# facebookresearch/PoseDiffusion

Measured on NVIDIA H100. Metric: diffusion steps/sec (20-frame seq, GGS on), higher is better.
Workload: dtype f32

## Files before the change

### posediffusion_b200/csrc/api_tc.cu

```cuda
#include <cuda.h>
#include <cudaTypedefs.h>

#include <algorithm>
#include <cstdint>
#include <cstdlib>

#include "context.cuh"
#include "tc_linear.cuh"

using namespace pdb;

namespace {

PFN_cuTensorMapEncodeTiled_v12000 get_encode() {
  static PFN_cuTensorMapEncodeTiled_v12000 fn = nullptr;
  if (!fn) {
    void* p = nullptr;
    cudaDriverEntryPointQueryResult qres;
    if (cudaGetDriverEntryPoint("cuTensorMapEncodeTiled", &p, cudaEnableDefault, &qres) == cudaSuccess &&
        qres == cudaDriverEntryPointSuccess)
      fn = reinterpret_cast<PFN_cuTensorMapEncodeTiled_v12000>(p);
  }
  return fn;
}
// ... 127 lines not shown
  return (long long)(O / 64) * ((S + kTcBM - 1) / kTcBM) <= ctx->sm_count && !getenv("PDB_TC_NO_SMALL");
}

}

extern "C" int pdb_debug_tc_linear(pdb_context* c, const float* x_dev, const float* w_dev, const float* bias_dev,
                                   const float* residual_dev, float* y_dev, int32_t S, int32_t O, int32_t K, int32_t relu,
                                   void* stream) {
  if (!c) return PDB_ERR_INVALID;
  Context* ctx = reinterpret_cast<Context*>(c);
  if (!x_dev || !w_dev || !y_dev) return ctx->fail(PDB_ERR_INVALID, "null argument");
  PDB_CUDA(ctx, cudaSetDevice(ctx->device));
  TcEpilogue E = {};
  E.bias = bias_dev;
  E.residual = residual_dev;
  E.ldr = O;
  E.Y = y_dev;
  E.ldy = O;
  E.S = S;
  E.O = O;
  E.K = K;
  E.relu = relu;
  E.allow_small = 1;
  return enqueue_tc_linear(ctx, x_dev, w_dev, E, static_cast<cudaStream_t>(stream));
}

#include "weights.cuh"

namespace {

__global__ void embed_kernel(const float* __restrict__ x, float* __restrict__ emb, int S) {
  pdl_trigger();
  pdl_wait();
  const int i = blockIdx.x * blockDim.x + threadIdx.x;
  if (i >= S * kPoseEmbPad) return;
  const int s = i / kPoseEmbPad, col = i - s * kPoseEmbPad;
  float v = 0.f;
  if (col < 180) {
    const int j = col < 90 ? col : col - 90;
    const int c = j / 10, k = j - c * 10;
    const float arg = x[s * 9 + c] * (float)(1 << k);
    v = col < 90 ? sinf(arg) : cosf(arg);
  } else if (col < kPoseEmb) {
    v = x[s * 9 + (col - 180)];
  }
  emb[i] = v;
}
__global__ void pivot_add_kernel(float* __restrict__ zproj, const float* __restrict__ w_pivot, int batch, int frames) {
  const int i = blockIdx.x * blockDim.x + threadIdx.x;
  if (i < batch * kDM) zproj[(size_t)(i / kDM) * frames * kDM + (i % kDM)] += w_pivot[i % kDM];
}
__global__ void row_stats_kernel(const float* __restrict__ h, float* __restrict__ mean, float* __restrict__ rstd, int S) {
  pdl_trigger();
  pdl_wait();
  const int row = blockIdx.x * (blockDim.x >> 5) + (threadIdx.x >> 5), lane = threadIdx.x & 31;
  if (row >= S) return;
  const float4* p = reinterpret_cast<const float4*>(h + (size_t)row * kDM);
  float4 v[4];
  float sum = 0.f;
#pragma unroll
  for (int i = 0; i < 4; ++i) {
    v[i] = p[lane + 32 * i];
    sum += v[i].x + v[i].y + v[i].z + v[i].w;
  }
  const float m = warp_sum(sum) * (1.0f / kDM);
  float sq = 0.f;
#pragma unroll
  for (int i = 0; i < 4; ++i) {
    const float a = v[i].x - m, b = v[i].y - m, c = v[i].z - m, d = v[i].w - m;
    sq += a * a + b * b + c * c + d * d;
  }
  const float var = warp_sum(sq) * (1.0f / kDM);
  if (lane == 0) {
    mean[row] = m;
    rstd[row] = 1.0f / sqrtf(var + kLnEps);
  }
}
__global__ void __launch_bounds__(kDenThreads) attention_kernel(const float* __restrict__ qkv, float* __restrict__ att, int frames) {
  extern __shared__ __align__(16) float att_smem[];
  pdl_trigger();
  pdl_wait();
  const int chunks = (frames + kDenWarps - 1) / kDenWarps;
  const int item = blockIdx.x;
  attention_item<false>(att_smem, qkv, att, item / (kHeads * chunks), (item / chunks) % kHeads, item % chunks, frames, 0u, 0u);
}
__global__ void __launch_bounds__(kDenThreads) tail_kernel(const __grid_constant__ DenoiserDev W, const __grid_constant__ DenoiserRun R, const int* __restrict__ tstate) {
  pdl_trigger();
  pdl_wait();
  const int s = blockIdx.x * kDenWarps + (threadIdx.x >> 5);
  const int t = tstate[0];
  if (s < R.tokens) tail_token<false>(W, R, s, t, t == tstate[1], 0u, 0u);
}
__global__ void step_set_kernel(int* tstate, int t, int t_lo) { tstate[0] = t; tstate[1] = t_lo; }
__global__ void step_dec_kernel(int* tstate) {
  pdl_wait();
  tstate[0] -= 1;
}

}

namespace pdb {

int enqueue_denoiser_tc(Context* ctx, DenoiserRun run, cudaStream_t st) {
  const DenoiserWeights* w = ctx->weights;
  const TcWeights& T = w->tc;
  const int S = run.tokens, B = run.batch, N = run.frames;
  const size_t need = sizeof(float) * (denoiser_ws_floats(S) + (size_t)S * (kPoseEmbPad + 2) + 64);
  if (int rc = ensure_buffer(ctx, &ctx->den_ws, &ctx->den_ws_bytes, need)) return rc;
  int* tstate = reinterpret_cast<int*>(ctx->den_ws) + 32;
  float* ws = static_cast<float*>(ctx->den_ws) + 64;
  run.zproj = ws; ws += (size_t)S * kDM;
  run.h = ws;     ws += (size_t)S * kDM;
  run.qkv = ws;   ws += (size_t)S * 3 * kDM;
  run.att = ws;   ws += (size_t)S * kDM;
  run.ff = ws;    ws += (size_t)S * kFF;
  run.u = ws;     ws += (size_t)S * kHid;
  float* emb = ws; ws += (size_t)S * kPoseEmbPad;
  float* mean = ws; ws += S;
  float* rstd = ws;
  bool pdl = false;
  auto lin = [&](const float* X, const float* Wm, int O, int K, const float* bias, const int* t_ptr, const float* residual, int ldr,
                 const float* colsum, float* Y, int relu, cudaStream_t s) {
    TcEpilogue E = {};
    E.bias = bias; E.t_ptr = t_ptr; E.bias_t_stride = kDM; E.residual = residual; E.ldr = ldr;
    E.colsum = colsum; E.row_mean = colsum ? mean : nullptr; E.row_rstd = colsum ? rstd : nullptr;
    E.Y = Y; E.ldy = O; E.S = S; E.O = O; E.K = K; E.relu = relu;
    E.allow_small = 1;
    E.pdl = pdl;
    E.stats = colsum && tc_linear_small(ctx, S, O);
    return enqueue_tc_linear(ctx, X, Wm, E, s);
  };
  const size_t att_smem = sizeof(float) * ((size_t)N * (kHD + 4) + (size_t)N * kHD + 2 * kDenWarps * kHD) + 64;
  size_t& att_attr = ctx->attr_att;
  if (att_smem > att_attr) {
    PDB_CUDA(ctx, cudaFuncSetAttribute(attention_kernel, cudaFuncAttributeMaxDynamicSharedMemorySize, (int)att_smem));
    att_attr = att_smem;
  }
  const int chunks = (N + kDenWarps - 1) / kDenWarps;
  const bool was_profiling = ctx->profiling;
  ScopedTimer total(ctx, st, 1);
  ctx->profiling = false;
  if (run.compute_zproj) {
    if (int rc = lin(run.z, T.wz, kDM, kZ, T.b_first, nullptr, nullptr, 0, nullptr, run.zproj, 0, st)) { ctx->profiling = was_profiling; return rc; }
    pivot_add_kernel<<<(B * kDM + 255) / 256, 256, 0, st>>>(run.zproj, T.w_pivot, B, N);
    ctx->launches += 1;
  }
  const bool stats_qkv = tc_linear_small(ctx, S, 3 * kDM), stats_ff1 = tc_linear_small(ctx, S, kFF);
  auto enqueue_step = [&](cudaStream_t s) -> int {
    pdl = ctx->tc_pdl && S <= 320;
    PDB_CUDA(ctx, launch_chained(embed_kernel, dim3((S * kPoseEmbPad + 255) / 256), dim3(256), 0, s, false, (const float*)run.x, emb, S));
    if (int rc = lin(emb, T.wx, kDM, kPoseEmbPad, T.tproj, tstate, run.zproj, kDM, nullptr, run.h, 0, s)) return rc;
    for (int l = 0; l < kLayers; ++l) {
      const TcLayer& L = T.layer[l];
      if (!stats_qkv) PDB_CUDA(ctx, launch_chained(row_stats_kernel, dim3((S + 7) / 8), dim3(256), 0, s, pdl, (const float*)run.h, mean, rstd, S));
      if (int rc = lin(run.h, L.wqkv, 3 * kDM, kDM, L.bias_qkv, nullptr, nullptr, 0, L.colsum_qkv, run.qkv, 0, s)) return rc;
      PDB_CUDA(ctx, launch_chained(attention_kernel, dim3(B * kHeads * chunks), dim3(kDenThreads), att_smem, s, pdl, (const float*)run.qkv, run.att, N));
      if (int rc = lin(run.att, L.wout, kDM, kDM, L.bout, nullptr, run.h, kDM, nullptr, run.h, 0, s)) return rc;
      if (!stats_ff1) PDB_CUDA(ctx, launch_chained(row_stats_kernel, dim3((S + 7) / 8), dim3(256), 0, s, pdl, (const float*)run.h, mean, rstd, S));
      if (int rc = lin(run.h, L.wff1, kFF, kDM, L.bias_ff1, nullptr, nullptr, 0, L.colsum_ff1, run.ff, 1, s)) return rc;
      if (int rc = lin(run.ff, L.wff2, kDM, kFF, L.bff2, nullptr, run.h, kDM, nullptr, run.h, 0, s)) return rc;
    }
    if (int rc = lin(run.h, T.wlast0, kHid, kDM, T.blast0, nullptr, nullptr, 0, nullptr, run.u, 0, s)) return rc;
    PDB_CUDA(ctx, launch_chained(tail_kernel, dim3((S + kDenWarps - 1) / kDenWarps), dim3(kDenThreads), 0, s, pdl, w->dev, run, (const int*)tstate));
    PDB_CUDA(ctx, launch_chained(step_dec_kernel, dim3(1), dim3(1), 0, s, pdl, tstate));
    pdl = false;
    return PDB_OK;
  };
// ... 63 lines not shown
```

### posediffusion_b200/csrc/common.cuh

```cuda
#pragma once
#include <cuda_runtime.h>
#include <stdint.h>

namespace pdb {

constexpr int kTargetDim = 9;
constexpr int kMaxFrames = 128;

__device__ __forceinline__ float warp_sum(float v) {
#pragma unroll
  for (int o = 16; o > 0; o >>= 1) v += __shfl_xor_sync(0xffffffffu, v, o);
  return v;
}

__device__ __forceinline__ float warp_reduce16(float (&v)[16], int lane) {
  {
    const bool hi = lane & 16;
#pragma unroll
    for (int i = 0; i < 8; ++i) {
      float send = hi ? v[i] : v[i + 8];
      float keep = hi ? v[i + 8] : v[i];
      v[i] = keep + __shfl_xor_sync(0xffffffffu, send, 16);
    }
  }
// ... 11 lines not shown
#pragma unroll
    for (int i = 0; i < 2; ++i) {
      float send = hi ? v[i] : v[i + 2];
      float keep = hi ? v[i + 2] : v[i];
      v[i] = keep + __shfl_xor_sync(0xffffffffu, send, 4);
    }
  }
  {
    const bool hi = lane & 2;
    float send = hi ? v[0] : v[1];
    float keep = hi ? v[1] : v[0];
    v[0] = keep + __shfl_xor_sync(0xffffffffu, send, 2);
  }
  v[0] += __shfl_xor_sync(0xffffffffu, v[0], 1);
  return v[0];
}
__device__ __forceinline__ int warp_reduce16_slot(int lane) {
  return ((lane >> 4) & 1) * 8 + ((lane >> 3) & 1) * 4 + ((lane >> 2) & 1) * 2 + ((lane >> 1) & 1);
}

#if defined(PDB_EMU) && defined(__CUDACC__)
#error "PDB_EMU is the CPU test harness of tests/host/cuda_emu.h; it must never be defined in an nvcc (product) build"
#endif
#ifdef PDB_EMU
inline float4 ld_stream_f4(const float4* p) { return *p; }
inline unsigned ld_acquire_u32(const unsigned* p) {
  sched_yield();
  return __atomic_load_n(p, __ATOMIC_ACQUIRE);
}
inline unsigned ld_relaxed_u32(const unsigned* p) { return __atomic_load_n(p, __ATOMIC_RELAXED); }
inline void red_release_add_u32(unsigned* p, unsigned v) { __atomic_fetch_add(p, v, __ATOMIC_RELEASE); }
inline void st_ll(unsigned long long* p, unsigned bits, unsigned tag) {
  __atomic_store_n(p, ((unsigned long long)tag << 32) | (unsigned long long)bits, __ATOMIC_RELAXED);
}
inline unsigned long long ld_ll(const unsigned long long* p) { return __atomic_load_n(p, __ATOMIC_RELAXED); }
inline void pdl_wait() {}
inline void pdl_trigger() {}
inline void ld_ll2(const unsigned long long* p, unsigned long long& a, unsigned long long& b) {
  a = __atomic_load_n(p, __ATOMIC_RELAXED);
  b = __atomic_load_n(p + 1, __ATOMIC_RELAXED);
}
inline void st_ll2(unsigned long long* p, unsigned bits0, unsigned bits1, unsigned tag) {
  st_ll(p, bits0, tag);
  st_ll(p + 1, bits1, tag);
}
inline void red_pair_add(float* p, float v) {
  unsigned long long* u = reinterpret_cast<unsigned long long*>(p);
  unsigned long long old = __atomic_load_n(u, __ATOMIC_RELAXED);
  for (;;) {
    float f[2];
    memcpy(f, &old, 8);
    f[0] += v;
    f[1] += 1.0f;
    unsigned long long want;
    memcpy(&want, f, 8);
    if (__atomic_compare_exchange_n(u, &old, want, false, __ATOMIC_RELAXED, __ATOMIC_RELAXED)) return;
  }
}
inline float2 ld_pair(const float* p) {
  const unsigned long long w = __atomic_load_n(reinterpret_cast<const unsigned long long*>(p), __ATOMIC_RELAXED);
  float f[2];
  memcpy(f, &w, 8);
  return make_float2(f[0], f[1]);
}
inline void st_pair_zero(float* p) { __atomic_store_n(reinterpret_cast<unsigned long long*>(p), 0ull, __ATOMIC_RELAXED); }
inline void red_add_u64(unsigned long long* p, unsigned long long v) { __atomic_fetch_add(p, v, __ATOMIC_RELAXED); }
inline void fence_gpu() { __atomic_thread_fence(__ATOMIC_SEQ_CST); }
inline void ll_backoff() {
  emu::yield();
  sched_yield();
}
inline uint32_t smem_u32(const void* p) { return emu::shared_addr(p); }
inline void mbar_init(uint32_t bar, uint32_t count) { emu::mbar_init(bar, count); }
inline void mbar_fence_init() {}
inline void mbar_arrive_expect_tx(uint32_t bar, uint32_t bytes) { emu::mbar_arrive_expect_tx(bar, bytes); }
inline bool mbar_try_wait(uint32_t bar, uint32_t parity) { return emu::mbar_try_wait(bar, parity); }
inline void mbar_wait(uint32_t bar, uint32_t parity) {
  while (!mbar_try_wait(bar, parity)) {
  }
}
inline void bulk_copy_g2s(uint32_t dst_smem, const void* src, uint32_t bytes, uint32_t bar) { emu::bulk_copy_g2s(dst_smem, src, bytes, bar); }
inline uint64_t l2_policy_evict_first() { return 0; }
inline void bulk_copy_g2s_hint(uint32_t dst_smem, const void* src, uint32_t bytes, uint32_t bar, uint64_t) { emu::bulk_copy_g2s(dst_smem, src, bytes, bar); }
#else
__device__ __forceinline__ float4 ld_stream_f4(const float4* p) {
  float4 r;
  asm volatile("ld.global.nc.L1::no_allocate.v4.f32 {%0,%1,%2,%3}, [%4];"
               : "=f"(r.x), "=f"(r.y), "=f"(r.z), "=f"(r.w)
               : "l"(p));
  return r;
}
__device__ __forceinline__ unsigned ld_acquire_u32(const unsigned* p) {
  unsigned v;
  asm volatile("ld.acquire.gpu.global.u32 %0, [%1];" : "=r"(v) : "l"(p) : "memory");
  return v;
}
__device__ __forceinline__ void red_release_add_u32(unsigned* p, unsigned v) {
  asm volatile("red.release.gpu.global.add.u32 [%0], %1;" ::"l"(p), "r"(v) : "memory");
}
__device__ __forceinline__ void st_ll(unsigned long long* p, unsigned bits, unsigned tag) {
  const unsigned long long w = ((unsigned long long)tag << 32) | (unsigned long long)bits;
  asm volatile("st.relaxed.gpu.global.b64 [%0], %1;" ::"l"(p), "l"(w) : "memory");
}
__device__ __forceinline__ unsigned long long ld_ll(const unsigned long long* p) {
  unsigned long long w;
  asm volatile("ld.relaxed.gpu.global.b64 %0, [%1];" : "=l"(w) : "l"(p) : "memory");
  return w;
}
__device__ __forceinline__ void pdl_wait() { asm volatile("griddepcontrol.wait;" ::: "memory"); }
__device__ __forceinline__ void pdl_trigger() { asm volatile("griddepcontrol.launch_dependents;" ::: "memory"); }
__device__ __forceinline__ void ld_ll2(const unsigned long long* p, unsigned long long& a, unsigned long long& b) {
  asm volatile("ld.relaxed.gpu.global.v2.b64 {%0,%1}, [%2];" : "=l"(a), "=l"(b) : "l"(p) : "memory");
}
__device__ __forceinline__ void st_ll2(unsigned long long* p, unsigned bits0, unsigned bits1, unsigned tag) {
  const unsigned long long w0 = ((unsigned long long)tag << 32) | (unsigned long long)bits0;
  const unsigned long long w1 = ((unsigned long long)tag << 32) | (unsigned long long)bits1;
  asm volatile("st.relaxed.gpu.global.v2.b64 [%0], {%1,%2};" ::"l"(p), "l"(w0), "l"(w1) : "memory");
}
__device__ __forceinline__ void ll_backoff() {}
__device__ __forceinline__ void red_pair_add(float* p, float v) {
  asm volatile("red.relaxed.gpu.global.add.v2.f32 [%0], {%1, %2};" ::"l"(p), "f"(v), "f"(1.0f) : "memory");
}
__device__ __forceinline__ float2 ld_pair(const float* p) {
  float2 v;
  asm volatile("ld.relaxed.gpu.global.v2.f32 {%0,%1}, [%2];" : "=f"(v.x), "=f"(v.y) : "l"(p) : "memory");
  return v;
}
__device__ __forceinline__ void st_pair_zero(float* p) {
  asm volatile("st.relaxed.gpu.global.b64 [%0], %1;" ::"l"(p), "l"(0ull) : "memory");
}
__device__ __forceinline__ void red_add_u64(unsigned long long* p, unsigned long long v) {
  asm volatile("red.relaxed.gpu.global.add.u64 [%0], %1;" ::"l"(p), "l"(v) : "memory");
}
__device__ __forceinline__ void fence_gpu() { __threadfence(); }

__device__ __forceinline__ uint32_t smem_u32(const void* p) { return (uint32_t)__cvta_generic_to_shared(p); }
__device__ __forceinline__ void mbar_init(uint32_t bar, uint32_t count) {
  asm volatile("mbarrier.init.shared::cta.b64 [%0], %1;" ::"r"(bar), "r"(count) : "memory");
}
__device__ __forceinline__ void mbar_fence_init() { asm volatile("fence.mbarrier_init.release.cluster;" ::: "memory"); }
__device__ __forceinline__ void mbar_arrive_expect_tx(uint32_t bar, uint32_t bytes) {
  asm volatile("mbarrier.arrive.expect_tx.shared::cta.b64 _, [%0], %1;" ::"r"(bar), "r"(bytes) : "memory");
}
__device__ __forceinline__ bool mbar_try_wait(uint32_t bar, uint32_t parity) {
  uint32_t ok;
  asm volatile("{\n\t.reg .pred p;\n\tmbarrier.try_wait.parity.shared::cta.b64 p, [%1], %2;\n\tselp.u32 %0, 1, 0, p;\n\t}"
               : "=r"(ok)
               : "r"(bar), "r"(parity)
               : "memory");
  return ok != 0;
}
__device__ __forceinline__ void mbar_wait(uint32_t bar, uint32_t parity) {
  while (!mbar_try_wait(bar, parity)) {
  }
}
__device__ __forceinline__ void bulk_copy_g2s(uint32_t dst_smem, const void* src, uint32_t bytes, uint32_t bar) {
  asm volatile("cp.async.bulk.shared::cluster.global.mbarrier::complete_tx::bytes [%0], [%1], %2, [%3];" ::"r"(dst_smem),
               "l"(src), "r"(bytes), "r"(bar)
               : "memory");
}
__device__ __forceinline__ uint64_t l2_policy_evict_first() {
  uint64_t p;
  asm volatile("createpolicy.fractional.L2::evict_first.b64 %0, 1.0;" : "=l"(p));
  return p;
}
__device__ __forceinline__ void bulk_copy_g2s_hint(uint32_t dst_smem, const void* src, uint32_t bytes, uint32_t bar, uint64_t policy) {
  asm volatile("cp.async.bulk.shared::cluster.global.mbarrier::complete_tx::bytes.L2::cache_hint [%0], [%1], %2, [%3], %4;" ::"r"(dst_smem),
               "l"(src), "r"(bytes), "r"(bar), "l"(policy)
               : "memory");
}
__device__ __forceinline__ unsigned ld_relaxed_u32(const unsigned* p) {
  unsigned v;
  asm volatile("ld.relaxed.gpu.global.u32 %0, [%1];" : "=r"(v) : "l"(p) : "memory");
  return v;
}
#endif

constexpr int kLlBatch = 16;
template <bool kInt>
__device__ __forceinline__ unsigned ll_sum(const unsigned long long* base, size_t stride, int count, unsigned tag) {
  float fsum = 0.f;
  int isum = 0;
  for (int c0 = 0; c0 < count; c0 += kLlBatch) {
    unsigned long long w[kLlBatch];
    bool ok;
    do {
      ok = true;
#pragma unroll
      for (int k = 0; k < kLlBatch; ++k) {
        w[k] = ld_ll(base + (size_t)min(c0 + k, count - 1) * stride);
        ok = ok && ((unsigned)(w[k] >> 32) == tag);
      }
      if (!ok) ll_backoff();
    } while (!ok);
#pragma unroll
    for (int k = 0; k < kLlBatch; ++k) {
      const bool in = c0 + k < count;
      if (kInt) isum += in ? (int)(unsigned)w[k] : 0;
      else fsum += in ? __uint_as_float((unsigned)w[k]) : 0.f;
    }
  }
  return kInt ? (unsigned)isum : __float_as_uint(fsum);
}

__device__ __forceinline__ void warp_group_barrier(unsigned* counter, unsigned target) {
  __syncwarp();
  if ((threadIdx.x & 31) == 0) {
    red_release_add_u32(counter, 1u);
    while (ld_acquire_u32(counter) < target) {
    }
  }
  __syncwarp();
}

}
```

### posediffusion_b200/csrc/denoiser.cuh

```cuda
#pragma once
#include <type_traits>

#include "common.cuh"
#include "posediff_b200.h"

namespace pdb {

constexpr int kDM = 512;
constexpr int kHeads = 4;
constexpr int kHD = 128;
constexpr int kFF = 1024;
constexpr int kLayers = 8;
constexpr int kHid = 128;
constexpr int kZ = 384;
constexpr int kTEmb = 128;
constexpr int kPoseEmb = 189;
constexpr int kPoseEmbPad = 256;
constexpr int kFirstIn = 702;
constexpr int kT = PDB_NUM_TIMESTEPS;
constexpr int kDenThreads = 256;
constexpr int kDenWarps = kDenThreads / 32;
constexpr float kLnEps = 1e-5f;

struct LayerWeights {
// ... 117 lines not shown
template <int K, int TS>
__device__ __forceinline__ void load_rows_flag(float* __restrict__ Xs, const unsigned long long* __restrict__ src, int row0,
                                               int valid_end, unsigned tag, const float* __restrict__ ln_g,
                                               const float* __restrict__ ln_b) {
  constexpr int K2 = K / 2;
  constexpr int TOTAL = TS * K2;
  constexpr int PER = (TOTAL + kDenThreads - 1) / kDenThreads;
  constexpr int ROUNDS = (PER + 19) / 20;
  constexpr int BATCH = (PER + ROUNDS - 1) / ROUNDS;
#pragma unroll 1
  for (int round = 0; round < ROUNDS; ++round) {
    unsigned long long a[BATCH], b[BATCH];
#pragma unroll
    for (int i = 0; i < BATCH; ++i) {
      const int idx = threadIdx.x + (round * BATCH + i) * kDenThreads;
      const int r = idx / K2, c = idx - r * K2;
      a[i] = b[i] = (unsigned long long)tag << 32;
      if (idx < TOTAL && row0 + r < valid_end) ld_ll2(src + (size_t)(row0 + r) * K + 2 * c, a[i], b[i]);
    }
#pragma unroll
    for (int i = 0; i < BATCH; ++i) {
      const int idx = threadIdx.x + (round * BATCH + i) * kDenThreads;
      const int r = idx / K2, c = idx - r * K2;
      if (idx < TOTAL) {
        while (!ll_ready(a[i], tag) || !ll_ready(b[i], tag)) {
          ll_backoff();
          ld_ll2(src + (size_t)(row0 + r) * K + 2 * c, a[i], b[i]);
        }
        reinterpret_cast<float2*>(Xs)[idx] = make_float2(ll_value(a[i]), ll_value(b[i]));
      }
    }
  }
  if (ln_g) {
    __syncthreads();
    layer_norm_rows<K, TS>(Xs, row0, valid_end, ln_g, ln_b);
  }
}

__device__ __forceinline__ void load_pose_embed(float* __restrict__ Xs, float* __restrict__ xrow, const float* __restrict__ x,
                                                const unsigned long long* __restrict__ fx, unsigned tag, int row0, int rows,
                                                int valid_end) {
  for (int i = threadIdx.x; i < rows * kTargetDim; i += kDenThreads) {
    const int r = i / kTargetDim, c = i - r * kTargetDim;
    const int s = row0 + r;
    float v = 0.f;
    if (s < valid_end) {
      if (fx) {
        unsigned long long w = ld_ll(fx + (size_t)s * 16 + c);
        while (!ll_ready(w, tag)) {
          ll_backoff();
          w = ld_ll(fx + (size_t)s * 16 + c);
        }
        v = ll_value(w);
      } else {
        v = __ldcg(x + (size_t)s * kTargetDim + c);
      }
    }
    xrow[i] = v;
  }
  __syncthreads();
  for (int i = threadIdx.x; i < rows * kPoseEmbPad; i += kDenThreads) {
    const int r = i / kPoseEmbPad, col = i - r * kPoseEmbPad;
    const int s = row0 + r;
    float v = 0.f;
    if (s < valid_end && col < kPoseEmb) {
      if (col < 180) {
        const int j = col < 90 ? col : col - 90;
        const int c = j / 10, k = j - c * 10;
        const float arg = xrow[r * kTargetDim + c] * (float)(1 << k);
        v = col < 90 ? sinf(arg) : cosf(arg);
      } else {
        v = xrow[r * kTargetDim + (col - 180)];
      }
    }
    Xs[i] = v;
  }
}

enum : int { kEpiNone = 0, kEpiRelu = 1, kEpiSilu = 2 };

constexpr int kFPI = 8;
constexpr int kSlices = kDenWarps * 4;

template <int K>
struct LinW {
  static constexpr int K4 = K / 4;
  static constexpr int PER = K4 / kSlices;
  static_assert(K4 % kSlices == 0 && PER >= 1 && PER <= 16, "K layout");
  float4 w[PER];
};

template <int K>
__device__ __forceinline__ void linear_prefetch(LinW<K>& W, const float4* __restrict__ Wp, int O, int o0) {
  const int lane = threadIdx.x & 31, warp = threadIdx.x >> 5;
  const int slice = warp * 4 + (lane >> 3);
  const float4* wp = Wp + (size_t)slice * O + o0 + (lane & 7);
#pragma unroll
  for (int i = 0; i < LinW<K>::PER; ++i) W.w[i] = __ldg(wp + (size_t)i * kSlices * O);
}

struct LinEpi {
  const float* bias;
  const void* add1;
  int ld1;
  bool add1_flag;
  const float* add2;
  const float* add_rs;
  const float* rs;
  void* Y;
  int ldy;
  bool y_flag;
  int epi;
  unsigned tag;
};

template <int TS, int K, bool kFlag>
__device__ __forceinline__ void linear_item(const LinW<K>& W, const float* __restrict__ Xs, float* __restrict__ red, int o0,
                                            const LinEpi& E, int row0, int valid_end) {
  static_assert(TS % 4 == 0 && TS <= 32, "token tile");
  const int lane = threadIdx.x & 31, warp = threadIdx.x >> 5;
  constexpr int PER = LinW<K>::PER;
  const int ks = lane >> 3, f = lane & 7;
  const int s_out = threadIdx.x >> 3, f_out = threadIdx.x & 7;
  const bool has_out = s_out < TS && (row0 + s_out) < valid_end;
  float epi_add = 0.f;
  if (has_out) {
    const int row = row0 + s_out, o = o0 + f_out;
    if (E.bias) epi_add += __ldg(E.bias + o);
    if (E.add1) {
      if (kFlag && E.add1_flag) epi_add += ll_value(ld_ll(static_cast<const unsigned long long*>(E.add1) + (size_t)row * E.ld1 + o));
      else epi_add += __ldcg(static_cast<const float*>(E.add1) + (size_t)row * E.ld1 + o);
    }
    if (E.add2) epi_add += __ldg(E.add2 + o);
    if (E.add_rs) epi_add += __ldg(E.add_rs + o) * E.rs[s_out];
  }
  float acc[TS];
#pragma unroll
  for (int s = 0; s < TS; ++s) acc[s] = 0.f;
  const float* xs = Xs + (warp * 4 + ks) * 4;
#pragma unroll
  for (int i = 0; i < PER; ++i) {
#pragma unroll
    for (int s = 0; s < TS; ++s) {
      const float4 xv = *reinterpret_cast<const float4*>(xs + s * K + i * kSlices * 4);
      acc[s] = fmaf(W.w[i].x, xv.x, fmaf(W.w[i].y, xv.y, fmaf(W.w[i].z, xv.z, fmaf(W.w[i].w, xv.w, acc[s]))));
    }
  }
  constexpr int Q = TS / 4;
  {
    const bool hi = ks & 2;
#pragma unroll
    for (int s = 0; s < TS / 2; ++s) {
      const float send = hi ? acc[s] : acc[s + TS / 2];
      const float keep = hi ? acc[s + TS / 2] : acc[s];
      acc[s] = keep + __shfl_xor_sync(0xffffffffu, send, 16);
    }
  }
  {
    const bool hi = ks & 1;
#pragma unroll
    for (int s = 0; s < Q; ++s) {
      const float send = hi ? acc[s] : acc[s + Q];
      const float keep = hi ? acc[s + Q] : acc[s];
      acc[s] = keep + __shfl_xor_sync(0xffffffffu, send, 8);
    }
  }
#pragma unroll
  for (int s = 0; s < Q; ++s) red[(warp * TS + ks * Q + s) * kFPI + f] = acc[s];
  __syncthreads();
  if (s_out < TS) {
    float v = 0.f;
#pragma unroll
    for (int wv = 0; wv < kDenWarps; ++wv) v += red[(wv * TS + s_out) * kFPI + f_out];
    if (has_out) {
      v += epi_add;
      if (E.epi == kEpiRelu) v = fmaxf(v, 0.f);
      else if (E.epi == kEpiSilu) v = v / (1.0f + expf(-v));
      const size_t at = (size_t)(row0 + s_out) * E.ldy + o0 + f_out;
      if (kFlag && E.y_flag) st_ll(static_cast<unsigned long long*>(E.Y) + at, __float_as_uint(v), E.tag);
      else static_cast<float*>(E.Y)[at] = v;
    }
  }
  __syncthreads();
}

__device__ __forceinline__ float4 ld_ll_f4(const unsigned long long* p, unsigned tag) {
  unsigned long long w0, w1, w2, w3;
  ld_ll2(p, w0, w1);
  ld_ll2(p + 2, w2, w3);
  while (!ll_ready(w0, tag) || !ll_ready(w1, tag) || !ll_ready(w2, tag) || !ll_ready(w3, tag)) {
    ll_backoff();
    ld_ll2(p, w0, w1);
    ld_ll2(p + 2, w2, w3);
  }
  return make_float4(ll_value(w0), ll_value(w1), ll_value(w2), ll_value(w3));
}

template <bool kFlag>
__device__ __forceinline__ void attention_item(float* __restrict__ smem, const void* __restrict__ qkv_any, void* __restrict__ att_any,
                                               int seq, int head, int chunk, int N, unsigned tag_in, unsigned tag_out) {
  const int lane = threadIdx.x & 31, warp = threadIdx.x >> 5;
  constexpr int KP = kHD + 4;
  float* Ks = smem;
  float* Vs = Ks + N * KP;
  float* Qs = Vs + N * kHD;
  float* Ps = Qs + kDenWarps * kHD;
  const int i = chunk * kDenWarps + warp;
  float4 qv = make_float4(0.f, 0.f, 0.f, 0.f);
  if constexpr (kFlag) {
    const unsigned long long* base = static_cast<const unsigned long long*>(qkv_any) + (size_t)seq * N * (3 * kDM) + head * kHD;
    const int total = N * (kHD / 4);
    for (int e0 = threadIdx.x; e0 < total; e0 += 4 * kDenThreads) {
      unsigned long long kw[4][4], vw[4][4];
#pragma unroll
      for (int u = 0; u < 4; ++u) {
        const int e = e0 + u * kDenThreads;
        if (e < total) {
          const int j = e / (kHD / 4), d4 = e - j * (kHD / 4);
          const unsigned long long* kp = base + (size_t)j * 3 * kDM + kDM + d4 * 4;
          const unsigned long long* vp = base + (size_t)j * 3 * kDM + 2 * kDM + d4 * 4;
          ld_ll2(kp, kw[u][0], kw[u][1]);
          ld_ll2(kp + 2, kw[u][2], kw[u][3]);
          ld_ll2(vp, vw[u][0], vw[u][1]);
          ld_ll2(vp + 2, vw[u][2], vw[u][3]);
        }
      }
#pragma unroll
      for (int u = 0; u < 4; ++u) {
        const int e = e0 + u * kDenThreads;
        if (e < total) {
          const int j = e / (kHD / 4), d4 = e - j * (kHD / 4);
          const unsigned long long* kp = base + (size_t)j * 3 * kDM + kDM + d4 * 4;
          const unsigned long long* vp = base + (size_t)j * 3 * kDM + 2 * kDM + d4 * 4;
          while (!ll_ready(kw[u][0], tag_in) || !ll_ready(kw[u][1], tag_in) || !ll_ready(kw[u][2], tag_in) || !ll_ready(kw[u][3], tag_in)) {
            ll_backoff();
            ld_ll2(kp, kw[u][0], kw[u][1]);
            ld_ll2(kp + 2, kw[u][2], kw[u][3]);
          }
          while (!ll_ready(vw[u][0], tag_in) || !ll_ready(vw[u][1], tag_in) || !ll_ready(vw[u][2], tag_in) || !ll_ready(vw[u][3], tag_in)) {
            ll_backoff();
            ld_ll2(vp, vw[u][0], vw[u][1]);
            ld_ll2(vp + 2, vw[u][2], vw[u][3]);
          }
          *reinterpret_cast<float4*>(Ks + j * KP + d4 * 4) = make_float4(ll_value(kw[u][0]), ll_value(kw[u][1]), ll_value(kw[u][2]), ll_value(kw[u][3]));
          *reinterpret_cast<float4*>(Vs + j * kHD + d4 * 4) = make_float4(ll_value(vw[u][0]), ll_value(vw[u][1]), ll_value(vw[u][2]), ll_value(vw[u][3]));
        }
      }
    }
    if (i < N) qv = ld_ll_f4(base + (size_t)i * 3 * kDM + lane * 4, tag_in);
  } else {
    const float* base = static_cast<const float*>(qkv_any) + (size_t)seq * N * (3 * kDM) + head * kHD;
    if (i < N) qv = __ldcg(reinterpret_cast<const float4*>(base + (size_t)i * 3 * kDM) + lane);
    for (int e = threadIdx.x; e < N * (kHD / 4); e += kDenThreads) {
      const int j = e / (kHD / 4), d4 = e - j * (kHD / 4);
      const float4 kv = __ldcg(reinterpret_cast<const float4*>(base + (size_t)j * 3 * kDM + kDM) + d4);
      const float4 vv = __ldcg(reinterpret_cast<const float4*>(base + (size_t)j * 3 * kDM + 2 * kDM) + d4);
      *reinterpret_cast<float4*>(Ks + j * KP + d4 * 4) = kv;
      *reinterpret_cast<float4*>(Vs + j * kHD + d4 * 4) = vv;
    }
  }
  const float scaling = 0.08838834764831845f;
  *reinterpret_cast<float4*>(Qs + warp * kHD + lane * 4) = make_float4(qv.x * scaling, qv.y * scaling, qv.z * scaling, qv.w * scaling);
  __syncthreads();
  if (i < N) {
    float sc[4];
    float mx = -INFINITY;
#pragma unroll
    for (int p = 0; p < 4; ++p) {
      const int j = p * 32 + lane;
      float dot = -INFINITY;
      if (p * 32 < N && j < N) {
        const float4* kr = reinterpret_cast<const float4*>(Ks + j * KP);
        const float4* qr = reinterpret_cast<const float4*>(Qs + warp * kHD);
        float d0 = 0.f, d1 = 0.f, d2 = 0.f, d3 = 0.f;
#pragma unroll 8
        for (int d = 0; d < kHD / 4; ++d) {
          const float4 a = qr[d], b = kr[d];
          d0 = fmaf(a.x, b.x, d0); d1 = fmaf(a.y, b.y, d1); d2 = fmaf(a.z, b.z, d2); d3 = fmaf(a.w, b.w, d3);
        }
        dot = (d0 + d1) + (d2 + d3);
      }
      sc[p] = dot;
      mx = fmaxf(mx, dot);
    }
#pragma unroll
    for (int o = 16; o > 0; o >>= 1) mx = fmaxf(mx, __shfl_xor_sync(0xffffffffu, mx, o));
    float sum = 0.f;
#pragma unroll
    for (int p = 0; p < 4; ++p) {
      const int j = p * 32 + lane;
      const float e = (j < N) ? expf(sc[p] - mx) : 0.f;
      sc[p] = e;
      sum += e;
    }
    sum = warp_sum(sum);
    const float inv = 1.0f / sum;
#pragma unroll
    for (int p = 0; p < 4; ++p) {
      const int j = p * 32 + lane;
      if (j < N) Ps[warp * kHD + j] = sc[p] * inv;
    }
    __syncwarp();
    float4 o4 = make_float4(0.f, 0.f, 0.f, 0.f);
    for (int j = 0; j < N; ++j) {
      const float pj = Ps[warp * kHD + j];
      const float4 vv = *reinterpret_cast<const float4*>(Vs + j * kHD + lane * 4);
      o4.x = fmaf(pj, vv.x, o4.x); o4.y = fmaf(pj, vv.y, o4.y); o4.z = fmaf(pj, vv.z, o4.z); o4.w = fmaf(pj, vv.w, o4.w);
    }
    const size_t at = ((size_t)seq * N + i) * kDM + head * kHD + lane * 4;
    if constexpr (kFlag) {
      unsigned long long* dst = static_cast<unsigned long long*>(att_any) + at;
      st_ll2(dst, __float_as_uint(o4.x), __float_as_uint(o4.y), tag_out);
      st_ll2(dst + 2, __float_as_uint(o4.z), __float_as_uint(o4.w), tag_out);
    } else {
      *reinterpret_cast<float4*>(static_cast<float*>(att_any) + at) = o4;
    }
  }
  __syncthreads();
}

template <bool kFlag>
__device__ __forceinline__ void tail_token(const DenoiserDev& W, const DenoiserRun& R, int s, int t, bool last_step, unsigned tag_u,
                                           unsigned tag_x) {
  const int lane = threadIdx.x & 31;
  float4 v;
  if constexpr (kFlag) v = ld_ll_f4(R.fu + (size_t)s * kHid + lane * 4, tag_u);
  else v = __ldcg(reinterpret_cast<const float4*>(R.u + (size_t)s * kHid) + lane);
  const float mean = warp_sum(v.x + v.y + v.z + v.w) * (1.0f / kHid);
  v.x -= mean; v.y -= mean; v.z -= mean; v.w -= mean;
  const float rstd = 1.0f / sqrtf(warp_sum(v.x * v.x + v.y * v.y + v.z * v.z + v.w * v.w) * (1.0f / kHid) + kLnEps);
  const float4 g = __ldg(reinterpret_cast<const float4*>(W.ln_last_g) + lane);
  const float4 b = __ldg(reinterpret_cast<const float4*>(W.ln_last_b) + lane);
  v.x = fmaxf(v.x * rstd * g.x + b.x, 0.f);
  v.y = fmaxf(v.y * rstd * g.y + b.y, 0.f);
  v.z = fmaxf(v.z * rstd * g.z + b.z, 0.f);
  v.w = fmaxf(v.w * rstd * g.w + b.w, 0.f);
  float mine = 0.f;
#pragma unroll
  for (int c = 0; c < kTargetDim; ++c) {
    const float4 w = __ldg(reinterpret_cast<const float4*>(W.w_last3 + c * kHid) + lane);
    const float dot = warp_sum(w.x * v.x + w.y * v.y + w.z * v.z + w.w * v.w);
    if (lane == c) mine = dot + __ldg(W.b_last3 + c);
  }
  if (lane < kTargetDim) {
    const float* sc = W.sched + t * 8;
    const size_t e = (size_t)s * kTargetDim + lane;
    const float xt = __ldcg(R.x + e);
    const float x0 = sc[0] * xt - sc[1] * mine;
    const float mu = sc[2] * x0 + sc[3] * xt;
    float out = mu;
    const int k = (kT - 1) - t;
    if (t >= R.guide_below && t > 0 && R.draws) out = mu + sc[4] * __ldg(R.draws + (size_t)(1 + k) * R.tokens * kTargetDim + e);
    R.x[e] = out;
    if constexpr (kFlag) st_ll(R.fx + (size_t)s * 16 + lane, __float_as_uint(out), tag_x);
    if (R.trail && t >= R.guide_below) R.trail[(size_t)(1 + k) * R.tokens * kTargetDim + e] = out;
    if (last_step) {
      if (R.eps_out) R.eps_out[e] = mine;
      if (R.x0_out) R.x0_out[e] = x0;
      if (R.mean_out) R.mean_out[e] = mu;
    }
  }
}

template <int TS, bool kFlag>
__global__ void __launch_bounds__(kDenThreads, 1)
denoiser_kernel(const __grid_constant__ DenoiserDev W, const __grid_constant__ DenoiserRun R) {
#ifdef PDB_EMU
  float* const smem = reinterpret_cast<float*>(emu::g_cta->smem);
#else
  extern __shared__ __align__(16) float smem[];
#endif
  float* Xs = smem;
  __shared__ float pivot[32];
  __shared__ float xrow[32 * kTargetDim];
  const int S = R.tokens;
  const int tiles = (S + TS - 1) / TS;
  const int G = gridDim.x;
  unsigned bar_count = 0;
  long long clk[5] = {0, 0, 0, 0, 0};
  const bool probe = R.dbg_clock != nullptr && threadIdx.x == 0;
  auto barrier = [&]() {
    if constexpr (!kFlag) {
      ++bar_count;
      long long c0 = 0;
      if (probe) c0 = clock64();
      __syncthreads();
      if (threadIdx.x == 0) {
        red_release_add_u32(R.bar, 1u);
        while (ld_acquire_u32(R.bar) < bar_count * (unsigned)G) {
        }
      }
      __syncthreads();
      if (probe) clk[0] += clock64() - c0;
    }
  };
  auto linear_stage = [&](auto ktag, const float4* Wp, int O, auto&& load_x, const LinEpi& E, bool need_barrier) {
    constexpr int K = decltype(ktag)::value;
    const int groups = O / kFPI;
    const int n_items = tiles * groups;
    LinW<K> wreg;
    int item = blockIdx.x;
    if (item < n_items) linear_prefetch<K>(wreg, Wp, O, (item % groups) * kFPI);
    if (need_barrier) barrier();
    float* red = Xs + TS * K;
    int staged_tile = -1;
    for (; item < n_items; item += G) {
      const int tt = item / groups, fg = item - tt * groups;
      if (item != (int)blockIdx.x) linear_prefetch<K>(wreg, Wp, O, fg * kFPI);
      long long c0 = 0, c1 = 0;
      if (probe) c0 = clock64();
      if (tt != staged_tile) {
        load_x(tt);
        staged_tile = tt;
      }
      __syncthreads();
      if (probe) c1 = clock64();
      linear_item<TS, K, kFlag>(wreg, Xs, red, fg * kFPI, E, tt * TS, S);
      if (probe) {
        clk[1] += c1 - c0;
        clk[2] += clock64() - c1;
      }
    }
  };
  void* const h_buf = kFlag ? static_cast<void*>(R.fh) : static_cast<void*>(R.h);
  void* const att_buf = kFlag ? static_cast<void*>(R.fatt) : static_cast<void*>(R.att);
  void* const ff_buf = kFlag ? static_cast<void*>(R.fff) : static_cast<void*>(R.ff);
  void* const u_buf = kFlag ? static_cast<void*>(R.fu) : static_cast<void*>(R.u);
  auto load_tile = [&](auto ktag, const void* src, int tt, unsigned tag, const float* g, const float* b) {
    constexpr int K = decltype(ktag)::value;
    if constexpr (kFlag) load_rows_flag<K, TS>(Xs, static_cast<const unsigned long long*>(src), tt * TS, S, tag, g, b);
    else load_rows<K, TS>(Xs, static_cast<const float*>(src), tt * TS, S, g, b);
  };
  using KDM = std::integral_constant<int, kDM>;
  using KFF = std::integral_constant<int, kFF>;
  bool pending = false;
  if (R.compute_zproj) {
    const LinEpi E = {W.b_first, nullptr, 0, false, nullptr, W.w_first_pivot, pivot, R.zproj, kDM, false, kEpiNone, 0u};
    linear_stage(std::integral_constant<int, kZ>{}, W.w_first_z, kDM,
                 [&](int tt) {
                   load_rows<kZ, TS>(Xs, R.z, tt * TS, S, nullptr, nullptr);
                   if (threadIdx.x < TS) pivot[threadIdx.x] = ((tt * TS + threadIdx.x) % R.frames == 0) ? 1.f : 0.f;
                 },
                 E, false);
    pending = true;
  }
  for (int t = R.t_hi; t >= R.t_lo; --t) {
    const unsigned v0 = R.tag_base + (unsigned)(R.t_hi - t) * kTagsPerStep;
    {
      const bool shadow = kFlag && t != R.t_hi;
      const LinEpi E = {nullptr, R.zproj, kDM, false, W.tproj + t * kDM, nullptr, nullptr, h_buf, kDM, kFlag, kEpiNone, v0};
      linear_stage(std::integral_constant<int, kPoseEmbPad>{}, W.w_first_x, kDM,
                   [&](int tt) { load_pose_embed(Xs, xrow, R.x, shadow ? R.fx : nullptr, v0 - kTagsPerStep + 42, tt * TS, TS, S); }, E,
                   pending);
    }
    pending = true;
    for (int l = 0; l < kLayers; ++l) {
      const LayerWeights& L = W.layer[l];
      const unsigned v_h_in = v0 + (l == 0 ? 0 : 5 * l), v_qkv = v0 + 1 + 5 * l, v_att = v0 + 2 + 5 * l, v_h_mid = v0 + 3 + 5 * l,
                     v_ff = v0 + 4 + 5 * l, v_h_out = v0 + 5 + 5 * l;
      void* const qkv_buf = kFlag ? static_cast<void*>(R.fqkv + (size_t)(l & 1) * S * 3 * kDM) : static_cast<void*>(R.qkv);
      {
        const LinEpi E = {L.b_qkv, nullptr, 0, false, nullptr, nullptr, nullptr, qkv_buf, 3 * kDM, kFlag, kEpiNone, v_qkv};
        linear_stage(KDM{}, L.w_qkv, 3 * kDM, [&](int tt) { load_tile(KDM{}, h_buf, tt, v_h_in, L.ln1_g, L.ln1_b); }, E, true);
      }
      barrier();
      {
        long long c0 = 0;
        if (probe) c0 = clock64();
        const int chunks = (R.frames + kDenWarps - 1) / kDenWarps;
        for (int item = blockIdx.x; item < R.batch * kHeads * chunks; item += G)
          attention_item<kFlag>(Xs, qkv_buf, att_buf, item / (kHeads * chunks), (item / chunks) % kHeads, item % chunks, R.frames,
                                v_qkv, v_att);
        if (probe) clk[3] += clock64() - c0;
      }
      {
        const LinEpi E = {L.b_out, h_buf, kDM, kFlag, nullptr, nullptr, nullptr, h_buf, kDM, kFlag, kEpiNone, v_h_mid};
        linear_stage(KDM{}, L.w_out, kDM, [&](int tt) { load_tile(KDM{}, att_buf, tt, v_att, nullptr, nullptr); }, E, true);
      }
      {
        const LinEpi E = {L.b_ff1, nullptr, 0, false, nullptr, nullptr, nullptr, ff_buf, kFF, kFlag, kEpiRelu, v_ff};
        linear_stage(KDM{}, L.w_ff1, kFF, [&](int tt) { load_tile(KDM{}, h_buf, tt, v_h_mid, L.ln2_g, L.ln2_b); }, E, true);
      }
      {
        const LinEpi E = {L.b_ff2, h_buf, kDM, kFlag, nullptr, nullptr, nullptr, h_buf, kDM, kFlag, kEpiNone, v_h_out};
        linear_stage(KFF{}, L.w_ff2, kDM, [&](int tt) { load_tile(KFF{}, ff_buf, tt, v_ff, nullptr, nullptr); }, E, true);
      }
    }
    {
      const LinEpi E = {W.b_last0, nullptr, 0, false, nullptr, nullptr, nullptr, u_buf, kHid, kFlag, kEpiNone, v0 + 41};
      linear_stage(KDM{}, W.w_last0, kHid, [&](int tt) { load_tile(KDM{}, h_buf, tt, v0 + 5 * kLayers, nullptr, nullptr); }, E, true);
    }
    barrier();
    {
      long long c0 = 0;
      if (probe) c0 = clock64();
      const int warp_global = blockIdx.x * kDenWarps + (threadIdx.x >> 5);
      for (int s = warp_global; s < S; s += G * kDenWarps) tail_token<kFlag>(W, R, s, t, t == R.t_lo, v0 + 41, v0 + 42);
      if (probe) clk[4] += clock64() - c0;
    }
    pending = true;
  }
  if (probe) {
    long long* c = R.dbg_clock + (size_t)blockIdx.x * 8;
    for (int k = 0; k < 5; ++k) c[k] += clk[k];
    c[5] += R.t_hi - R.t_lo + 1;
  }
}

inline size_t denoiser_smem_bytes(int TS, int frames) {
  size_t lin = (size_t)TS * kFF + (size_t)kDenWarps * TS * kFPI;
  size_t att = (size_t)frames * (kHD + 4) + (size_t)frames * kHD + 2 * kDenWarps * kHD;
  return sizeof(float) * (lin > att ? lin : att) + 256;
}

}
```

Before: 1311.

## Stream denoiser weights through a cp.async shared-memory ring across stages and barriers

Replaces per-item register prefetch of linear weights with a two-slot shared-memory ring filled by cp.async. A cursor walks ahead across linear stages and timesteps, so the next weights load while barriers, attention and the current matmul run. It also adapts the attention rows per block to the grid size so more blocks get work, and batches the K/V global loads for more memory-level parallelism. The cost is extra shared memory (two 32 KB slots), which may reduce occupancy, plus a cursor that must stay in step with the stage schedule.

```diff
diff --git a/posediffusion_b200/csrc/api_tc.cu b/posediffusion_b200/csrc/api_tc.cu
--- a/posediffusion_b200/csrc/api_tc.cu
+++ b/posediffusion_b200/csrc/api_tc.cu
@@ -233,7 +233,7 @@
   pdl_wait();
   const int chunks = (frames + kDenWarps - 1) / kDenWarps;
   const int item = blockIdx.x;
-  attention_item<false>(att_smem, qkv, att, item / (kHeads * chunks), (item / chunks) % kHeads, item % chunks, frames, 0u, 0u);
+  attention_item<false>(att_smem, qkv, att, item / (kHeads * chunks), (item / chunks) % kHeads, item % chunks, kDenWarps, frames, 0u, 0u);
 }
 __global__ void __launch_bounds__(kDenThreads) tail_kernel(const __grid_constant__ DenoiserDev W, const __grid_constant__ DenoiserRun R, const int* __restrict__ tstate) {
   pdl_trigger();
diff --git a/posediffusion_b200/csrc/common.cuh b/posediffusion_b200/csrc/common.cuh
--- a/posediffusion_b200/csrc/common.cuh
+++ b/posediffusion_b200/csrc/common.cuh
@@ -117,6 +117,10 @@
 inline void bulk_copy_g2s(uint32_t dst_smem, const void* src, uint32_t bytes, uint32_t bar) { emu::bulk_copy_g2s(dst_smem, src, bytes, bar); }
 inline uint64_t l2_policy_evict_first() { return 0; }
 inline void bulk_copy_g2s_hint(uint32_t dst_smem, const void* src, uint32_t bytes, uint32_t bar, uint64_t) { emu::bulk_copy_g2s(dst_smem, src, bytes, bar); }
+inline void cp_async_16_hint(void* dst_smem, const void* src, uint64_t) { memcpy(dst_smem, src, 16); }
+inline void cp_async_commit() {}
+template <int N>
+inline void cp_async_wait() {}
 #else
 __device__ __forceinline__ float4 ld_stream_f4(const float4* p) {
   float4 r;
@@ -203,6 +207,15 @@
   asm volatile("cp.async.bulk.shared::cluster.global.mbarrier::complete_tx::bytes.L2::cache_hint [%0], [%1], %2, [%3], %4;" ::"r"(dst_smem),
                "l"(src), "r"(bytes), "r"(bar), "l"(policy)
                : "memory");
+}
+__device__ __forceinline__ void cp_async_16_hint(void* dst_smem, const void* src, uint64_t policy) {
+  asm volatile("cp.async.cg.shared.global.L2::cache_hint [%0], [%1], 16, %2;" ::"r"(smem_u32(dst_smem)), "l"(src), "l"(policy)
+               : "memory");
+}
+__device__ __forceinline__ void cp_async_commit() { asm volatile("cp.async.commit_group;" ::: "memory"); }
+template <int N>
+__device__ __forceinline__ void cp_async_wait() {
+  asm volatile("cp.async.wait_group %0;" ::"n"(N) : "memory");
 }
 __device__ __forceinline__ unsigned ld_relaxed_u32(const unsigned* p) {
   unsigned v;
diff --git a/posediffusion_b200/csrc/denoiser.cuh b/posediffusion_b200/csrc/denoiser.cuh
--- a/posediffusion_b200/csrc/denoiser.cuh
+++ b/posediffusion_b200/csrc/denoiser.cuh
@@ -223,21 +223,49 @@
 constexpr int kFPI = 8;
 constexpr int kSlices = kDenWarps * 4;
 
-template <int K>
-struct LinW {
-  static constexpr int K4 = K / 4;
-  static constexpr int PER = K4 / kSlices;
-  static_assert(K4 % kSlices == 0 && PER >= 1 && PER <= 16, "K layout");
-  float4 w[PER];
+constexpr int kDenLinStages = 2 + 4 * kLayers;
+constexpr int kWRing = 2;
+constexpr int kWSlotF4 = kFF / 4 * kFPI;
+
+struct DenStageW {
+  const float4* w;
+  int O, K;
 };
-
-template <int K>
-__device__ __forceinline__ void linear_prefetch(LinW<K>& W, const float4* __restrict__ Wp, int O, int o0) {
-  const int lane = threadIdx.x & 31, warp = threadIdx.x >> 5;
-  const int slice = warp * 4 + (lane >> 3);
-  const float4* wp = Wp + (size_t)slice * O + o0 + (lane & 7);
-#pragma unroll
-  for (int i = 0; i < LinW<K>::PER; ++i) W.w[i] = __ldg(wp + (size_t)i * kSlices * O);
+__device__ __forceinline__ DenStageW den_stage_weights(const DenoiserDev& W, int id) {
+  if (id == 0) return {W.w_first_z, kDM, kZ};
+  if (id == 1) return {W.w_first_x, kDM, kPoseEmbPad};
+  if (id == kDenLinStages) return {W.w_last0, kHid, kDM};
+  const LayerWeights& L = W.layer[(id - 2) >> 2];
+  switch ((id - 2) & 3) {
+    case 0: return {L.w_qkv, 3 * kDM, kDM};
+    case 1: return {L.w_out, kDM, kDM};
+    case 2: return {L.w_ff1, kFF, kDM};
+    default: return {L.w_ff2, kDM, kFF};
+  }
+}
+
+struct WeightCursor {
+  int t, id, item;
+};
+__device__ __forceinline__ void wc_settle(WeightCursor& c, const DenoiserDev& W, int t_lo, int tiles) {
+  while (c.t >= t_lo && c.item >= tiles * (den_stage_weights(W, c.id).O / kFPI)) {
+    c.item = blockIdx.x;
+    if (++c.id > kDenLinStages) {
+      c.id = 1;
+      --c.t;
+    }
+  }
+}
+__device__ __forceinline__ void wc_issue(WeightCursor& c, const DenoiserDev& W, int t_lo, int tiles, float4* slot) {
+  if (c.t >= t_lo) {
+    const DenStageW s = den_stage_weights(W, c.id);
+    const float4* src = s.w + (size_t)(c.item % (s.O / kFPI)) * kFPI;
+    const uint64_t policy = l2_policy_evict_first();
+    for (int e = threadIdx.x; e < s.K / 4 * kFPI; e += kDenThreads) cp_async_16_hint(slot + e, src + (size_t)(e / kFPI) * s.O + e % kFPI, policy);
+    c.item += gridDim.x;
+    wc_settle(c, W, t_lo, tiles);
+  }
+  cp_async_commit();
 }
 
 struct LinEpi {
@@ -256,11 +284,12 @@
 };
 
 template <int TS, int K, bool kFlag>
-__device__ __forceinline__ void linear_item(const LinW<K>& W, const float* __restrict__ Xs, float* __restrict__ red, int o0,
+__device__ __forceinline__ void linear_item(const float4* __restrict__ Ws, const float* __restrict__ Xs, float* __restrict__ red, int o0,
                                             const LinEpi& E, int row0, int valid_end) {
   static_assert(TS % 4 == 0 && TS <= 32, "token tile");
+  static_assert(K / 4 % kSlices == 0 && K / 4 * kFPI <= kWSlotF4, "K layout");
   const int lane = threadIdx.x & 31, warp = threadIdx.x >> 5;
-  constexpr int PER = LinW<K>::PER;
+  constexpr int PER = K / 4 / kSlices;
   const int ks = lane >> 3, f = lane & 7;
   const int s_out = threadIdx.x >> 3, f_out = threadIdx.x & 7;
   const bool has_out = s_out < TS && (row0 + s_out) < valid_end;
@@ -279,12 +308,14 @@
 #pragma unroll
   for (int s = 0; s < TS; ++s) acc[s] = 0.f;
   const float* xs = Xs + (warp * 4 + ks) * 4;
+  const float4* ws = Ws + (warp * 4 + ks) * kFPI + f;
 #pragma unroll
   for (int i = 0; i < PER; ++i) {
+    const float4 w = ws[i * kSlices * kFPI];
 #pragma unroll
     for (int s = 0; s < TS; ++s) {
       const float4 xv = *reinterpret_cast<const float4*>(xs + s * K + i * kSlices * 4);
-      acc[s] = fmaf(W.w[i].x, xv.x, fmaf(W.w[i].y, xv.y, fmaf(W.w[i].z, xv.z, fmaf(W.w[i].w, xv.w, acc[s]))));
+      acc[s] = fmaf(w.x, xv.x, fmaf(w.y, xv.y, fmaf(w.z, xv.z, fmaf(w.w, xv.w, acc[s]))));
     }
   }
   constexpr int Q = TS / 4;
@@ -339,14 +370,14 @@
 
 template <bool kFlag>
 __device__ __forceinline__ void attention_item(float* __restrict__ smem, const void* __restrict__ qkv_any, void* __restrict__ att_any,
-                                               int seq, int head, int chunk, int N, unsigned tag_in, unsigned tag_out) {
+                                               int seq, int head, int chunk, int rows, int N, unsigned tag_in, unsigned tag_out) {
   const int lane = threadIdx.x & 31, warp = threadIdx.x >> 5;
   constexpr int KP = kHD + 4;
   float* Ks = smem;
   float* Vs = Ks + N * KP;
   float* Qs = Vs + N * kHD;
   float* Ps = Qs + kDenWarps * kHD;
-  const int i = chunk * kDenWarps + warp;
+  const int i = warp < rows ? chunk * rows + warp : N;
   float4 qv = make_float4(0.f, 0.f, 0.f, 0.f);
   if constexpr (kFlag) {
     const unsigned long long* base = static_cast<const unsigned long long*>(qkv_any) + (size_t)seq * N * (3 * kDM) + head * kHD;
@@ -392,12 +423,27 @@
   } else {
     const float* base = static_cast<const float*>(qkv_any) + (size_t)seq * N * (3 * kDM) + head * kHD;
     if (i < N) qv = __ldcg(reinterpret_cast<const float4*>(base + (size_t)i * 3 * kDM) + lane);
-    for (int e = threadIdx.x; e < N * (kHD / 4); e += kDenThreads) {
-      const int j = e / (kHD / 4), d4 = e - j * (kHD / 4);
-      const float4 kv = __ldcg(reinterpret_cast<const float4*>(base + (size_t)j * 3 * kDM + kDM) + d4);
-      const float4 vv = __ldcg(reinterpret_cast<const float4*>(base + (size_t)j * 3 * kDM + 2 * kDM) + d4);
-      *reinterpret_cast<float4*>(Ks + j * KP + d4 * 4) = kv;
-      *reinterpret_cast<float4*>(Vs + j * kHD + d4 * 4) = vv;
+    const int total = N * (kHD / 4);
+    for (int e0 = threadIdx.x; e0 < total; e0 += 4 * kDenThreads) {
+      float4 kv[4], vv[4];
+#pragma unroll
+      for (int u = 0; u < 4; ++u) {
+        const int e = e0 + u * kDenThreads;
+        if (e < total) {
+          const int j = e / (kHD / 4), d4 = e - j * (kHD / 4);
+          kv[u] = __ldcg(reinterpret_cast<const float4*>(base + (size_t)j * 3 * kDM + kDM) + d4);
+          vv[u] = __ldcg(reinterpret_cast<const float4*>(base + (size_t)j * 3 * kDM + 2 * kDM) + d4);
+        }
+      }
+#pragma unroll
+      for (int u = 0; u < 4; ++u) {
+        const int e = e0 + u * kDenThreads;
+        if (e < total) {
+          const int j = e / (kHD / 4), d4 = e - j * (kHD / 4);
+          *reinterpret_cast<float4*>(Ks + j * KP + d4 * 4) = kv[u];
+          *reinterpret_cast<float4*>(Vs + j * kHD + d4 * 4) = vv[u];
+        }
+      }
     }
   }
   const float scaling = 0.08838834764831845f;
@@ -501,6 +547,15 @@
       if (R.mean_out) R.mean_out[e] = mu;
     }
   }
+}
+
+__host__ __device__ inline size_t denoiser_ring_offset(int TS, int frames) {
+  const size_t lin = (size_t)TS * kFF + (size_t)kDenWarps * TS * kFPI;
+  const size_t att = (size_t)frames * (kHD + 4) + (size_t)frames * kHD + 2 * kDenWarps * kHD;
+  return (sizeof(float) * (lin > att ? lin : att) + 127) / 128 * 128;
+}
+inline size_t denoiser_smem_bytes(int TS, int frames) {
+  return denoiser_ring_offset(TS, frames) + (size_t)kWRing * kWSlotF4 * sizeof(float4);
 }
 
 template <int TS, bool kFlag>
@@ -535,28 +590,33 @@
       if (probe) clk[0] += clock64() - c0;
     }
   };
-  auto linear_stage = [&](auto ktag, const float4* Wp, int O, auto&& load_x, const LinEpi& E, bool need_barrier) {
+  float4* const wring = reinterpret_cast<float4*>(reinterpret_cast<unsigned char*>(smem) + denoiser_ring_offset(TS, R.frames));
+  WeightCursor wc = {R.t_hi, R.compute_zproj ? 0 : 1, (int)blockIdx.x};
+  unsigned w_used = 0;
+  wc_settle(wc, W, R.t_lo, tiles);
+  for (int s = 0; s < kWRing; ++s) wc_issue(wc, W, R.t_lo, tiles, wring + s * kWSlotF4);
+  auto linear_stage = [&](auto ktag, int id, auto&& load_x, const LinEpi& E, bool need_barrier) {
     constexpr int K = decltype(ktag)::value;
-    const int groups = O / kFPI;
+    const int groups = den_stage_weights(W, id).O / kFPI;
     const int n_items = tiles * groups;
-    LinW<K> wreg;
-    int item = blockIdx.x;
-    if (item < n_items) linear_prefetch<K>(wreg, Wp, O, (item % groups) * kFPI);
     if (need_barrier) barrier();
     float* red = Xs + TS * K;
     int staged_tile = -1;
-    for (; item < n_items; item += G) {
+    for (int item = blockIdx.x; item < n_items; item += G) {
       const int tt = item / groups, fg = item - tt * groups;
-      if (item != (int)blockIdx.x) linear_prefetch<K>(wreg, Wp, O, fg * kFPI);
       long long c0 = 0, c1 = 0;
       if (probe) c0 = clock64();
       if (tt != staged_tile) {
         load_x(tt);
         staged_tile = tt;
       }
+      cp_async_wait<kWRing - 1>();
       __syncthreads();
       if (probe) c1 = clock64();
-      linear_item<TS, K, kFlag>(wreg, Xs, red, fg * kFPI, E, tt * TS, S);
+      float4* const slot = wring + (w_used % kWRing) * kWSlotF4;
+      linear_item<TS, K, kFlag>(slot, Xs, red, fg * kFPI, E, tt * TS, S);
+      wc_issue(wc, W, R.t_lo, tiles, slot);
+      ++w_used;
       if (probe) {
         clk[1] += c1 - c0;
         clk[2] += clock64() - c1;
@@ -574,10 +634,12 @@
   };
   using KDM = std::integral_constant<int, kDM>;
   using KFF = std::integral_constant<int, kFF>;
+  const int att_rows = min(kDenWarps, max(1, (R.batch * kHeads * R.frames + G - 1) / G));
+  const int att_chunks = (R.frames + att_rows - 1) / att_rows;
   bool pending = false;
   if (R.compute_zproj) {
     const LinEpi E = {W.b_first, nullptr, 0, false, nullptr, W.w_first_pivot, pivot, R.zproj, kDM, false, kEpiNone, 0u};
-    linear_stage(std::integral_constant<int, kZ>{}, W.w_first_z, kDM,
+    linear_stage(std::integral_constant<int, kZ>{}, 0,
                  [&](int tt) {
                    load_rows<kZ, TS>(Xs, R.z, tt * TS, S, nullptr, nullptr);
                    if (threadIdx.x < TS) pivot[threadIdx.x] = ((tt * TS + threadIdx.x) % R.frames == 0) ? 1.f : 0.f;
@@ -590,7 +652,7 @@
     {
       const bool shadow = kFlag && t != R.t_hi;
       const LinEpi E = {nullptr, R.zproj, kDM, false, W.tproj + t * kDM, nullptr, nullptr, h_buf, kDM, kFlag, kEpiNone, v0};
-      linear_stage(std::integral_constant<int, kPoseEmbPad>{}, W.w_first_x, kDM,
+      linear_stage(std::integral_constant<int, kPoseEmbPad>{}, 1,
                    [&](int tt) { load_pose_embed(Xs, xrow, R.x, shadow ? R.fx : nullptr, v0 - kTagsPerStep + 42, tt * TS, TS, S); }, E,
                    pending);
     }
@@ -602,34 +664,33 @@
       void* const qkv_buf = kFlag ? static_cast<void*>(R.fqkv + (size_t)(l & 1) * S * 3 * kDM) : static_cast<void*>(R.qkv);
       {
         const LinEpi E = {L.b_qkv, nullptr, 0, false, nullptr, nullptr, nullptr, qkv_buf, 3 * kDM, kFlag, kEpiNone, v_qkv};
-        linear_stage(KDM{}, L.w_qkv, 3 * kDM, [&](int tt) { load_tile(KDM{}, h_buf, tt, v_h_in, L.ln1_g, L.ln1_b); }, E, true);
+        linear_stage(KDM{}, 2 + 4 * l, [&](int tt) { load_tile(KDM{}, h_buf, tt, v_h_in, L.ln1_g, L.ln1_b); }, E, true);
       }
       barrier();
       {
         long long c0 = 0;
         if (probe) c0 = clock64();
-        const int chunks = (R.frames + kDenWarps - 1) / kDenWarps;
-        for (int item = blockIdx.x; item < R.batch * kHeads * chunks; item += G)
-          attention_item<kFlag>(Xs, qkv_buf, att_buf, item / (kHeads * chunks), (item / chunks) % kHeads, item % chunks, R.frames,
-                                v_qkv, v_att);
+        for (int item = blockIdx.x; item < R.batch * kHeads * att_chunks; item += G)
+          attention_item<kFlag>(Xs, qkv_buf, att_buf, item / (kHeads * att_chunks), (item / att_chunks) % kHeads, item % att_chunks,
+                                att_rows, R.frames, v_qkv, v_att);
         if (probe) clk[3] += clock64() - c0;
       }
       {
         const LinEpi E = {L.b_out, h_buf, kDM, kFlag, nullptr, nullptr, nullptr, h_buf, kDM, kFlag, kEpiNone, v_h_mid};
-        linear_stage(KDM{}, L.w_out, kDM, [&](int tt) { load_tile(KDM{}, att_buf, tt, v_att, nullptr, nullptr); }, E, true);
+        linear_stage(KDM{}, 3 + 4 * l, [&](int tt) { load_tile(KDM{}, att_buf, tt, v_att, nullptr, nullptr); }, E, true);
       }
       {
         const LinEpi E = {L.b_ff1, nullptr, 0, false, nullptr, nullptr, nullptr, ff_buf, kFF, kFlag, kEpiRelu, v_ff};
-        linear_stage(KDM{}, L.w_ff1, kFF, [&](int tt) { load_tile(KDM{}, h_buf, tt, v_h_mid, L.ln2_g, L.ln2_b); }, E, true);
+        linear_stage(KDM{}, 4 + 4 * l, [&](int tt) { load_tile(KDM{}, h_buf, tt, v_h_mid, L.ln2_g, L.ln2_b); }, E, true);
       }
       {
         const LinEpi E = {L.b_ff2, h_buf, kDM, kFlag, nullptr, nullptr, nullptr, h_buf, kDM, kFlag, kEpiNone, v_h_out};
-        linear_stage(KFF{}, L.w_ff2, kDM, [&](int tt) { load_tile(KFF{}, ff_buf, tt, v_ff, nullptr, nullptr); }, E, true);
+        linear_stage(KFF{}, 5 + 4 * l, [&](int tt) { load_tile(KFF{}, ff_buf, tt, v_ff, nullptr, nullptr); }, E, true);
       }
     }
     {
       const LinEpi E = {W.b_last0, nullptr, 0, false, nullptr, nullptr, nullptr, u_buf, kHid, kFlag, kEpiNone, v0 + 41};
-      linear_stage(KDM{}, W.w_last0, kHid, [&](int tt) { load_tile(KDM{}, h_buf, tt, v0 + 5 * kLayers, nullptr, nullptr); }, E, true);
+      linear_stage(KDM{}, kDenLinStages, [&](int tt) { load_tile(KDM{}, h_buf, tt, v0 + 5 * kLayers, nullptr, nullptr); }, E, true);
     }
     barrier();
     {
@@ -648,10 +709,4 @@
   }
 }
 
-inline size_t denoiser_smem_bytes(int TS, int frames) {
-  size_t lin = (size_t)TS * kFF + (size_t)kDenWarps * TS * kFPI;
-  size_t att = (size_t)frames * (kHD + 4) + (size_t)frames * kHD + 2 * kDenWarps * kHD;
-  return sizeof(float) * (lin > att ? lin : att) + 256;
-}
-
-}
+}
```

Result: no change. 1324 (median of 6 runs) (+1.0%).
